# RmSchaffert/ACCV-Lab

Measured on AMD Instinct MI355X. Metric: heatmap frames/sec (1920x1080 fp32, ragged N_obj in [1,128], fused clear+draw), higher is better.
Workload: dtype f32

## Files before the change

### accv-lab_amd/accvlab/_amd_native/__init__.py

```python
from __future__ import annotations

import ctypes
import os

_HERE = os.path.dirname(os.path.abspath(__file__))
NO_HOST_FASTPATH = os.environ.get("ACCV_NO_HOST_FASTPATH", "") not in ("", "0")
LIB_PATH = os.environ.get("ACCV_HIP_LIB") or os.path.join(_HERE, "libaccv_hip.so")

OK = 0
HM_CLEAR = 1
HM_COUNTS_I64 = 2
HM_SMALL_RADII = 4
HM_WRITE_THROUGH = 8
HM_GROUP_BOXES_GIVEN = 16
HM_TILE_ROWS_16 = 32
HM_TILE_ROWS_8 = 64
HM_CALLER_SCALE_ORDER = 256
HM_PLAIN_STORES = 128
HM_POINT_COUNTS_I64 = 512
MP_IDX_I64 = 1
MP_COUNTS_I64 = 2
MP_LABELS_I64 = 4
FL_AVG_NUM_POS = 0
FL_AVG_VALUE = 1
FL_AVG_DEVICE = 2
LSA_MAXIMIZE = 1
LSA_THREADS_64 = 2
LSA_THREADS_1024 = 4
MC_ONE_MINUS_PROB = 0
MC_NEG_PROB = 1
MC_FOCAL = 2
MC_LABELS_I64 = 1
MC_CXCYWH = 2
CR_MAX_MAPS = 8
CR_MAX_CHANNELS = 64
CR_COUNTS_I64 = 1
CR_INDEX_FORM = 2
CR_WEIGHTS_PER_CHANNEL = 4
CR_L1 = 0
CR_SMOOTH_L1 = 2
MF_IDX_I64 = 1
MF_LABELS_I64 = 2
MB_IDX_I64 = 1
MB_CXCYWH = 2
MB_IOU_NONE = 0
MB_IOU = 1
MB_GIOU = 2
MB_MAX_D = 16
PM_IDX_I64 = 1
PM_REVERSIBLE = 2
PM_LABELS_I64 = 4
PM_CLOSED_I32 = 8
PM_CLOSED_I64 = 16
PM_MIN_P = 2
PM_MAX_P = 128
CT_MAX_TASKS = 8
CT_MAX_CLASSES = 64
CT_NO_TASK = 255
CT_LABELS_I64 = 1
CT_COUNTS_I64 = 2
BA_MAX_POINT_TRANSFORMS = 4
BA_MAX_FRAME_TRANSFORMS = 2
BA_COUNTS_I64 = 1
BA_LABELS_I64 = 2
BA_RANGE_ON_OUTPUT = 4
CD_MAX_TASKS = 8
CD_MAX_MAPS = 8
CD_MAX_CLASSES = 64
CD_MAX_K = 1024
RN_MAX_TASKS = 8
RN_MAX_N = 1024
RN_MIN_D = 7
RN_MAX_D = 16
VB_MAX_BOXES = 256
VB_COUNTS_I64 = 1
VB_HW_I64 = 2
CB_MAX_BOXES = 256
CB_MAX_MATRICES = 4
CB_COUNTS_I64 = 1
CB_HW_I64 = 2
CB_CATEGORIES_I64 = 4
BH_MAX_BOXES = 256
BH_MAX_CATEGORIES = 128
BH_TILE_W = 64
BH_TILE_H = 16
BH_COUNTS_I64 = 1
BH_HW_I64 = 2
BH_CATEGORIES_I64 = 4
IP_MAX_EXTENT = 16384
IP_TILE_W = 64
IP_TILE_H = 16
IP_LAYOUT_CHW = 0
IP_LAYOUT_HWC = 1

_vp = ctypes.c_void_p
_i = ctypes.c_int
_f = ctypes.c_float
_u = ctypes.c_uint
_sz = ctypes.c_size_t
_i64 = ctypes.c_int64
_ll = ctypes.c_longlong
_u64 = ctypes.c_uint64
# ... 381 lines not shown
```

### accv-lab_amd/accvlab/draw_heatmap/ops.py

```python
from __future__ import annotations

import ctypes
from typing import Optional

import torch

from .. import _amd_native as _nat

try:
    from . import _dh_host as _dh
except ImportError:
    _dh = None
_native_bound = False


def _native():
    global _native_bound
    if _dh is None or _nat.NO_HOST_FASTPATH:
        return None
    if not _native_bound:
        h = _nat.ctypes_lib()
        addr = lambda name: ctypes.cast(getattr(h, name), ctypes.c_void_p).value
        _dh.bind_native(addr("accv_draw_heatmap_batched_f32"), addr("accv_last_error"))
        _native_bound = True
    return _dh


_FORCED_FLAGS = 0


def _hint_flags(clear: bool, small_radii: bool, write_through: bool, tile_rows) -> int:
    if tile_rows not in (None, 8, 16):
        raise RuntimeError("tile_rows must be None, 8 or 16")
    return (_nat.HM_CLEAR if clear else 0) | (_nat.HM_SMALL_RADII if small_radii else 0) | \
        (0 if write_through is None else _nat.HM_WRITE_THROUGH if write_through else _nat.HM_PLAIN_STORES) | \
        (_nat.HM_TILE_ROWS_16 if tile_rows == 16 else _nat.HM_TILE_ROWS_8 if tile_rows == 8 else 0) | _FORCED_FLAGS


def _one_launch_maps(maps, batch: int, device):
    k = len(maps)
    if not 1 <= k <= 4:
        return None
    ptrs, hs, ws = [], [], []
    for hm in maps:
        if not (isinstance(hm, torch.Tensor) and hm.is_cuda and hm.dtype == torch.float32 and hm.is_contiguous() and
                hm.device == device):
            return None
        shape = hm.shape
        if len(shape) != 3 or shape[0] != batch:
            return None
        ptr = hm.data_ptr()
        if shape[2] % 4 or ptr % 16 or shape[1] * shape[2] * 4 >= (1 << 31):
            return None
        ptrs.append(ptr)
        hs.append(shape[1])
        ws.append(shape[2])
    return (ctypes.c_void_p * k)(*ptrs), (ctypes.c_int * k)(*hs), (ctypes.c_int * k)(*ws)


def _check_maps(maps, batch: int, device, owner: str) -> None:
    for hm in maps:
        _check_input(hm, "heatmap")
        _check_dtype(hm, torch.float32, "heatmap")
        if not (hm.dim() == 3 and hm.size(0) == batch):
            raise RuntimeError("every heatmap must be of shape [batch_size, height, width]")
        if not (hm.device == device):
            raise RuntimeError(f"every heatmap must be on the {owner}' device ({device})")


def _require(cond: bool, msg: str) -> None:
    if not cond:
        raise RuntimeError(msg)


def _check_input(t: torch.Tensor, name: str) -> None:
    if not (isinstance(t, torch.Tensor)):
        raise RuntimeError(f"{name} must be a torch.Tensor")
    if not (t.is_cuda):
        raise RuntimeError(f"{name} must be a CUDA tensor")
    if not (t.is_contiguous()):
        raise RuntimeError(f"{name} must be contiguous")


def _check_dtype(t: torch.Tensor, dtype: torch.dtype, name: str) -> None:
    if not (t.dtype == dtype):
        raise RuntimeError(f"{name}: expected scalar type {dtype} but found {t.dtype}")


def _same_device(ref: torch.Tensor, *others) -> None:
    for name, t in others:
        if not (t.device == ref.device):
            raise RuntimeError(f"{name} must be on the same device as the heatmap ({ref.device})")


_FLAT_DIRECT_MAX_OBJECTS = 2048
_FLAT_DIRECT_MAX_ROUNDS = 200_000
_constants: dict = {}


def _flat_direct(planes: int, height: int, width: int, n: int) -> bool:
    if not (0 < n <= _FLAT_DIRECT_MAX_OBJECTS and 0 < planes <= 65535 and height > 0 and width > 0):
        return False
    tiles = planes * ((width + 127) // 128) * ((height + 15) // 16)
    return tiles * ((n + 63) // 64) <= _FLAT_DIRECT_MAX_ROUNDS


def _device_constant(key, make) -> torch.Tensor:
    t = _constants.get(key)
    if t is None:
        t = make()
        if torch.cuda.is_current_stream_capturing():
            return t
        torch.cuda.current_stream(t.device).synchronize()
        if len(_constants) > 256:
            _constants.clear()
        _constants[key] = t
    return t


def draw_heatmap(
    heatmaps: torch.Tensor,
    centers: torch.Tensor,
    radii: torch.Tensor,
    heatmap_idxes: torch.Tensor,
    diameter_to_sigma_factor: float = 6.0,
    k_scale: float = 1.0,
    *,
    clear: bool = False,
    small_radii: bool = False,
    write_through: Optional[bool] = None,
    tile_rows: Optional[int] = None,
) -> None:
    _check_input(heatmaps, "heatmap")
    _check_input(centers, "centers")
    _check_input(radii, "radii")
    _check_input(heatmap_idxes, "heatmap_idxes")
    if not (centers.size(0) == radii.size(0)):
        raise RuntimeError("centers and radii must have the same size at dim0")
    if not (centers.size(0) == heatmap_idxes.size(0)):
        raise RuntimeError("centers and heatmap_idxes must have the same size at dim0")
    if not (heatmaps.dim() == 3):
        raise RuntimeError("heatmap must be of shape [num_heatmaps, height, width]")
    if not (centers.dim() == 2 and centers.size(1) == 2):
        raise RuntimeError("centers must be of shape [num_targets, 2]")
    if not (radii.dim() == 1 and heatmap_idxes.dim() == 1):
        raise RuntimeError("radii and heatmap_idxes must be of shape [num_targets]")
    _check_dtype(heatmaps, torch.float32, "heatmap")
    _check_dtype(centers, torch.int32, "centers")
    _check_dtype(radii, torch.int32, "radii")
    _check_dtype(heatmap_idxes, torch.int32, "heatmap_idxes")
    _same_device(heatmaps, ("centers", centers), ("radii", radii), ("heatmap_idxes", heatmap_idxes))

    lib = _nat.lib()
    planes, height, width = heatmaps.shape
    n = centers.size(0)
    if _flat_direct(planes, height, width, n):
        with _nat.device_guard(heatmaps.device):
            dev = heatmaps.device
            count = _device_constant(("count", n, dev), lambda: torch.full((1,), n, dtype=torch.int32, device=dev))
            status = lib.accv_draw_heatmap_batched_f32(
                heatmaps.data_ptr(), 1, planes, height, width, centers.data_ptr(), radii.data_ptr(), count.data_ptr(),
                heatmap_idxes.data_ptr(), n, float(diameter_to_sigma_factor), float(k_scale),
                _hint_flags(clear, small_radii, write_through, tile_rows), _nat.stream_ptr(heatmaps.device))
        _nat.check(status, "draw_heatmap")
        return
    with _nat.device_guard(heatmaps.device):
        ws_bytes = lib.accv_draw_heatmap_flat_workspace_bytes(planes, n)
        ws = torch.empty(ws_bytes, dtype=torch.uint8, device=heatmaps.device)
        status = lib.accv_draw_heatmap_flat_f32(
            heatmaps.data_ptr(), planes, height, width, centers.data_ptr(), radii.data_ptr(),
            heatmap_idxes.data_ptr(), n, float(diameter_to_sigma_factor), float(k_scale),
            _hint_flags(clear, small_radii, write_through, tile_rows), ws.data_ptr(), ws_bytes,
            _nat.stream_ptr(heatmaps.device))
    _nat.check(status, "draw_heatmap")


def draw_heatmap_batched(
    heatmap: torch.Tensor,
    centers,
    radii,
    diameter_to_sigma_factor: float = 6.0,
    k_scale: float = 1.0,
    labels=None,
    *,
    clear: bool = False,
    small_radii: bool = False,
    write_through: Optional[bool] = None,
    tile_rows: Optional[int] = None,
) -> None:
    centers_t = centers.tensor
    radii_t = radii.tensor
    assert centers_t.shape[0] == radii_t.shape[0], "centers and radii must have the same size batch size"
    assert centers_t.shape[1] == radii_t.shape[1], "centers and radii must have the same maximum number of objects"
    counts = centers.sample_sizes
    labels_t: Optional[torch.Tensor] = None
    if labels is not None:
        labels_t = labels.tensor
        assert centers_t.shape[0] == labels_t.shape[0], "centers and labels must have the same size batch size"
        assert centers_t.shape[1] == labels_t.shape[1], \
            "centers and labels must have the same maximum number of objects"

    native = _native()
    if native is not None and isinstance(heatmap, torch.Tensor) and isinstance(counts, torch.Tensor) and \
            native.draw_batched(heatmap, centers_t, radii_t, counts, labels_t, float(diameter_to_sigma_factor), float(k_scale),
                                _hint_flags(clear, small_radii, write_through, tile_rows)):
        return

    if counts.dtype not in (torch.int32, torch.int64):
        counts = counts.to(torch.int64)

    _check_input(heatmap, "heatmap")
    _check_input(centers_t, "centers")
    _check_input(radii_t, "radii")
    _check_input(counts, "nums_targets")
    batch = heatmap.size(0)
    n_max = radii_t.size(1) if radii_t.dim() >= 2 else -1
    _require(batch == radii_t.size(0) and batch == centers_t.size(0) and batch == counts.size(0),
             "batch_size (dim 0) need to be the same for all inputs")
    if not (centers_t.dim() == 3 and centers_t.size(2) == 2):
        raise RuntimeError("centers must be of shape [batch_size, num_targets, 2]")
    if not (radii_t.dim() == 2):
        raise RuntimeError("radii must be of shape [batch_size, num_targets]")
    if not (n_max == centers_t.size(1)):
        raise RuntimeError("maximum number of targets (dim 1) need to be the same centers and radii")
    if not (counts.dim() == 1):
        raise RuntimeError("nums_targets must be of shape [batch_size]")
    _check_dtype(heatmap, torch.float32, "heatmap")
    _check_dtype(centers_t, torch.int32, "centers")
    _check_dtype(radii_t, torch.int32, "radii")
    others = [("centers", centers_t), ("radii", radii_t), ("nums_targets", counts)]
    if labels_t is None:
        if not (heatmap.dim() == 3):
            raise RuntimeError("heatmap must be of shape [batch_size, height, width]")
        num_classes, (height, width) = 0, heatmap.shape[1:]
        labels_ptr = None
    else:
        _check_input(labels_t, "labels")
        if not (heatmap.dim() == 4):
            raise RuntimeError("heatmap must be of shape [batch_size, max_num_classes, height, width]")
        if not (labels_t.dim() == 2):
            raise RuntimeError("labels must be of shape [batch_size, radii.size(1)]")
        _require(labels_t.size(0) == batch and labels_t.size(1) == n_max,
                 "labels shape must be [batch_size, radii.size(1)]")
        _check_dtype(labels_t, torch.int32, "labels")
        num_classes, height, width = heatmap.shape[1:]
        if not (num_classes > 0 or heatmap.numel() == 0):
            raise RuntimeError("class-wise heatmap needs at least one class plane")
        labels_ptr = labels_t.data_ptr()
        others.append(("labels", labels_t))
    _same_device(heatmap, *others)
    if labels_t is not None and num_classes == 0:
        return

    flags = _hint_flags(clear, small_radii, write_through, tile_rows) | \
        (_nat.HM_COUNTS_I64 if counts.dtype == torch.int64 else 0)
    with _nat.device_guard(heatmap.device):
        status = _nat.lib().accv_draw_heatmap_batched_f32(
            heatmap.data_ptr(), batch, num_classes, height, width, centers_t.data_ptr(), radii_t.data_ptr(),
            counts.data_ptr(), labels_ptr, n_max, float(diameter_to_sigma_factor), float(k_scale), flags,
            _nat.stream_ptr(heatmap.device))
    _nat.check(status, "draw_heatmap_batched")


def get_centers_and_radii(centers, bboxes, out_size_factor: float):
    ragged = hasattr(centers, "tensor") and hasattr(centers, "create_with_sample_sizes_like_self")
    c_t = centers.tensor if ragged else centers
    b_t = bboxes.tensor if hasattr(bboxes, "tensor") else bboxes
    _require(c_t.shape[-1] == 2 and b_t.shape[-1] == 4 and c_t.shape[:-1] == b_t.shape[:-1],
             "centers must be [..., 2] and bboxes [..., 4] with equal leading dimensions")
    if c_t.is_cuda:
        if not (b_t.device == c_t.device):
            raise RuntimeError("centers and bboxes must be on the same device")
        c32 = c_t.to(torch.float32).contiguous()
        b32 = b_t.to(torch.float32).contiguous()
        out_c = torch.empty(c32.shape, dtype=torch.int32, device=c32.device)
        out_r = torch.empty(c32.shape[:-1], dtype=torch.int32, device=c32.device)
        with _nat.device_guard(c32.device):
            _nat.check(_nat.lib().accv_heatmap_targets_from_boxes_f32(
                c32.data_ptr(), b32.data_ptr(), out_r.numel(), float(out_size_factor), out_c.data_ptr(),
                out_r.data_ptr(), _nat.stream_ptr(c32.device)), "get_centers_and_radii")
    else:
        d = torch.cat([c_t - b_t[..., :2], b_t[..., 2:] - c_t], dim=-1)
        out_r = torch.ceil(torch.min(d, dim=-1)[0] / out_size_factor).to(torch.int32).clamp_(min=1)
        out_c = (c_t / out_size_factor).to(torch.int32)
    if ragged:
        nu = centers.non_uniform_dim
        return centers.create_with_sample_sizes_like_self(out_c, nu), centers.create_with_sample_sizes_like_self(out_r, nu)
    return out_c, out_r


def draw_heatmap_multiscale(heatmaps, centers, bboxes, out_size_factors, diameter_to_sigma_factor: float = 6.0,
                            k_scale: float = 1.0, *, clear: bool = False) -> None:
    heatmaps = list(heatmaps)
    strides = [float(f) for f in out_size_factors]
    if not (len(heatmaps) == len(strides) and len(heatmaps) >= 1):
        raise RuntimeError("heatmaps and out_size_factors must have the same, non-zero length")
    objects = _box_objects(centers, bboxes)
    batch, dev = objects[0].size(0), objects[0].device
    geometry = _one_launch_maps(heatmaps, batch, dev)
    if geometry is None:
        _check_maps(heatmaps, batch, dev, "centers")
        for hm, f in zip(heatmaps, strides):
            ci, ri = get_centers_and_radii(centers, bboxes, f)
            draw_heatmap_batched(hm, ci, ri, diameter_to_sigma_factor, k_scale, clear=clear)
        return
    _launch_box_maps(geometry, strides, objects, diameter_to_sigma_factor, k_scale, clear)


def _box_objects(centers, bboxes):
    c_t = centers.tensor
    b_t = bboxes.tensor if hasattr(bboxes, "tensor") else bboxes
    counts = centers.sample_sizes
    if counts.dtype not in (torch.int32, torch.int64):
        counts = counts.to(torch.int64)
    _check_input(c_t, "centers")
    _check_input(b_t, "bboxes")
    _check_input(counts, "nums_targets")
    if not (c_t.dim() == 3 and c_t.size(2) == 2):
        raise RuntimeError("centers must be of shape [batch_size, num_targets, 2]")
    if not (b_t.dim() == 3 and b_t.size(2) == 4 and b_t.shape[:2] == c_t.shape[:2]):
        raise RuntimeError("bboxes must be of shape [batch_size, num_targets, 4]")
    _check_dtype(c_t, torch.float32, "centers")
    _check_dtype(b_t, torch.float32, "bboxes")
    if not (counts.dim() == 1 and counts.size(0) == c_t.size(0)):
        raise RuntimeError("nums_targets must be of shape [batch_size]")
    _same_device(c_t, ("bboxes", b_t), ("nums_targets", counts))
    return c_t, b_t, counts


def _launch_box_maps(geometry, strides, objects, diameter_to_sigma_factor, k_scale, clear, job=None) -> None:
    ptrs, hs, ws = geometry
    c_t, b_t, counts = objects
    batch, n_max = c_t.shape[:2]
    n = len(strides)
    st = (ctypes.c_float * n)(*strides)
    flags = (_nat.HM_CLEAR if clear else 0) | (_nat.HM_COUNTS_I64 if counts.dtype == torch.int64 else 0) | _FORCED_FLAGS
    dev = c_t.device
# ... 13 lines not shown
```

### accv-lab_amd/csrc/draw_heatmap.hip

```cpp
#include <hip/hip_runtime.h>
#include <hip/hip_ext.h>

#include <algorithm>
#include <atomic>
#include <climits>
#include <cstdint>
#include <cstring>
#include <type_traits>

#include "accv_common.h"
#include "splat_common.h"
#include "splat_stamps.h"
#include "splat_tile.h"
#include "splat_small.h"
#include "splat_lanes.h"
#include "heatmap_prep.h"

namespace {

void note_dispatch(const char* kernel, int px, int r, bool clear, int sm, const dim3& grid, const dim3& block)
{
    snprintf(accv::dispatch_buffer(), 256, "%s<PX=%d,R=%d,CLEAR=%d,SM=%d> grid(%u,%u,%u) block(%u)", kernel, px, r, clear ? 1 : 0,
             sm, grid.x, grid.y, grid.z, block.x);
}

struct LaunchEvents {
    hipEvent_t start = nullptr, stop = nullptr;
};
LaunchEvents& launch_events()
{
    static thread_local LaunchEvents ev;
    return ev;
}
LaunchEvents take_launch_events()
{
    const LaunchEvents ev = launch_events();
    launch_events() = LaunchEvents{};
    return ev;
}
template <class K>
inline void launch_maybe_timed(K kernel, const dim3& grid, const dim3& block, hipStream_t stream, const LaunchEvents& ev,
                               const SplatParams& p)
{
    if (ev.start || ev.stop)
        hipExtLaunchKernelGGL(kernel, grid, block, 0, stream, ev.start, ev.stop, 0, p);
    else
        hipLaunchKernelGGL(kernel, grid, block, 0, stream, p);
}
template <class F>
void with_variant(bool clear, bool write_through, F&& f)
{
    using Plain = std::integral_constant<int, kStorePlain>;
    using WriteThrough = std::integral_constant<int, kStoreWriteThrough>;
    if (clear && write_through)
        f(std::true_type{}, WriteThrough{});
    else if (clear)
        f(std::true_type{}, Plain{});
    else if (write_through)
        f(std::false_type{}, WriteThrough{});
    else
        f(std::false_type{}, Plain{});
}

int launch_splat_small(SplatParams p, long long planes, bool clear, bool write_through, hipStream_t stream, const LaunchEvents& ev)
{
    p.tiles_x = (p.W + 127) / 128;
    p.tiles_y = (p.H + 15) / 16;
    p.n_tiles = planes * p.tiles_x * p.tiles_y;
    if (p.n_tiles == 0) return ACCV_OK;
    dim3 grid;
    p.grid3d = (planes <= 65535 && p.tiles_y <= 65535) ? 1 : 0;
    if (p.grid3d) {
        grid = dim3((unsigned)p.tiles_x, (unsigned)p.tiles_y, (unsigned)planes);
    } else {
        if (p.n_tiles > INT_MAX) return accv::fail(ACCV_EINVAL, "draw_heatmap: %lld tiles exceed the grid limit", p.n_tiles);
        grid = dim3((unsigned)p.n_tiles);
    }
    with_variant(clear, write_through, [&](auto CL, auto SM) {
        launch_maybe_timed(splat_small_kernel<CL, SM>, grid, dim3(64), stream, ev, p);
    });
    note_dispatch("splat_small_kernel", 4, 8, clear, write_through ? kStoreWriteThrough : kStorePlain, grid, dim3(64));
    return accv::check_launch("draw_heatmap small-splat kernel");
}

template <int PX, int R>
int launch_splat(SplatParams p, long long planes, bool clear, int sm, hipStream_t stream, const LaunchEvents& ev)
{
    p.tiles_x = (p.W + 32 * PX - 1) / (32 * PX);
    p.tiles_y = (p.H + 2 * R - 1) / (2 * R);
    p.n_tiles = planes * p.tiles_x * p.tiles_y;
    if (p.n_tiles == 0) return ACCV_OK;
    const int groups_x = (p.tiles_x + kWavesPerGroup - 1) / kWavesPerGroup;
    dim3 grid, block(kWavesPerGroup * 64);
    p.grid3d = (planes <= 65535 && p.tiles_y <= 65535) ? 1 : 0;
    if (p.grid3d) {
        grid = dim3((unsigned)groups_x, (unsigned)p.tiles_y, (unsigned)planes);
    } else {
        const long long groups = (p.n_tiles + kWavesPerGroup - 1) / kWavesPerGroup;
        if (groups > INT_MAX) return accv::fail(ACCV_EINVAL, "draw_heatmap: %lld tiles exceed the grid limit", p.n_tiles);
        grid = dim3((unsigned)groups);
    }
    attach_splat_stamps(p);
    if (PX == 1 || (sm == kStoreAdaptive && clear)) sm = kStorePlain;
    if (sm == kStoreAdaptive) {
        if constexpr (PX == 4) launch_maybe_timed(splat_kernel<PX, R, false, kStoreAdaptive>, grid, block, stream, ev, p);
    } else {
        with_variant(clear, sm == kStoreWriteThrough, [&](auto CL, auto SM) {
            if constexpr (PX == 4 || SM == kStorePlain) launch_maybe_timed(splat_kernel<PX, R, CL, SM>, grid, block, stream, ev, p);
        });
    }
    note_dispatch("splat_kernel", PX, R, clear, sm, grid, block);
    return accv::check_launch("draw_heatmap splat kernel");
}

long long compute_units()
{
    static std::atomic<int> cached[64];
    int dev = 0;
    if (hipGetDevice(&dev) != hipSuccess || dev < 0 || dev >= 64) return 0;
    int v = cached[dev].load(std::memory_order_relaxed);
    if (v == 0) {
        int n = 0;
        if (hipDeviceGetAttribute(&n, hipDeviceAttributeMultiprocessorCount, dev) != hipSuccess || n <= 0) return 0;
        cached[dev].store(n, std::memory_order_relaxed);
        v = n;
    }
    return v;
}

int dispatch_splat(SplatParams p, long long planes, bool clear, unsigned flags, hipStream_t stream, const LaunchEvents& ev)
{
    const bool small_hint = (flags & ACCV_HM_SMALL_RADII) != 0;
    const bool vec4 = (p.W % 4 == 0) && ((reinterpret_cast<uintptr_t>(p.hm) & 15u) == 0);
    const bool plane_fits_rsrc = (size_t)p.H * p.W * sizeof(float) < ((size_t)1 << 31);
    int nt;
    if (flags & ACCV_HM_WRITE_THROUGH)
        nt = kStoreWriteThrough;
    else if (flags & ACCV_HM_PLAIN_STORES)
        nt = kStorePlain;
    else
        nt = clear ? kStorePlain : kStoreAdaptive;
    if (nt != kStorePlain && !plane_fits_rsrc) nt = kStorePlain;
    p.dense_area = 0.75f * (float)p.H * (float)p.W;
    int rows = (flags & ACCV_HM_TILE_ROWS_16) ? 16 : 8;
    if (!(flags & (ACCV_HM_TILE_ROWS_8 | ACCV_HM_TILE_ROWS_16)) && clear && vec4 && !small_hint) {
        const long long cus = compute_units();
        const long long tx = (p.W + 127) / 128;
        const long long tiles8 = planes * tx * ((p.H + 15) / 16), tiles16 = planes * tx * ((p.H + 31) / 32);
        if (cus > 0 && tiles8 > 24 * cus && tiles16 <= 16 * cus) rows = 16;
    }
    if (!p.labels) p.labels = p.radii;
    if (!vec4) return launch_splat<1, 8>(p, planes, clear, kStorePlain, stream, ev);
    if (small_hint) return launch_splat_small(p, planes, clear, nt == kStoreWriteThrough, stream, ev);
    if (rows == 16) return launch_splat<4, 16>(p, planes, clear, nt, stream, ev);
    return launch_splat<4, 8>(p, planes, clear, nt, stream, ev);
}

int check_common(int h, int w, const char* who)
{
    if (h < 0 || w < 0) return accv::fail(ACCV_EINVAL, "%s: negative heatmap extent %dx%d", who, h, w);
    if (h > (1 << 29) || w > (1 << 29))
        return accv::fail(ACCV_EINVAL, "%s: heatmap extent %dx%d exceeds 2^29 per dimension", who, h, w);
    return ACCV_OK;
}

inline void coarse_scales_first(MultiParams& mp)
{
    std::stable_sort(mp.scale, mp.scale + mp.n_scales,
                     [](const SplatParams& a, const SplatParams& b) { return a.n_tiles < b.n_tiles; });
    long long tiles = 0;
    for (int i = 0; i < mp.n_scales; ++i) {
        mp.tile_begin[i] = tiles;
        tiles += mp.scale[i].n_tiles;
    }
    mp.tile_begin[mp.n_scales] = tiles;
}
inline void seal_tile_prefix(MultiParams& mp)
{
    for (int i = mp.n_scales + 1; i <= kMaxScales; ++i) mp.tile_begin[i] = mp.tile_begin[mp.n_scales];
}

inline int multiscale_store_mode(unsigned flags) { return (flags & ACCV_HM_WRITE_THROUGH) ? kStoreWriteThrough : kStorePlain; }

constexpr const char* kPerScaleNote = " (use the per-scale calls otherwise)";
long long setup_scales(MultiParams& mp, const SplatParams& proto, float* const* heatmaps, const int* heights, const int* widths,
                       const float* strides, int num_scales, int batch, int tile_h, unsigned flags, const char* who,
                       const char* map_note)
{
    long long tiles = 0;
    int used = 0;
    for (int i = 0; i < num_scales; ++i) {
        if (int rc = check_common(heights[i], widths[i], who)) return rc;
        if (!(strides[i] > 0.0f)) return accv::fail(ACCV_EINVAL, "%s: stride %d is not positive", who, i);
        if (heights[i] == 0 || widths[i] == 0) continue;
        if (!heatmaps[i]) return accv::fail(ACCV_EINVAL, "%s: heatmap %d is null", who, i);
        if (widths[i] % 4 != 0 || (reinterpret_cast<uintptr_t>(heatmaps[i]) & 15u) ||
            (size_t)heights[i] * widths[i] * sizeof(float) >= ((size_t)1 << 31))
            return accv::fail(ACCV_EINVAL, "%s: map %d needs a width that is a multiple of 4, a 16-byte aligned base and planes "
                                           "below 2 GiB%s", who, i, map_note);
        SplatParams& p = mp.scale[used];
        p = proto;
        p.hm = heatmaps[i];
        p.H = heights[i];
        p.W = widths[i];
        p.stride = strides[i];
        p.tiles_x = (p.W + 127) / 128;
        p.tiles_y = (p.H + tile_h - 1) / tile_h;
        p.n_tiles = (long long)batch * p.tiles_x * p.tiles_y;
        p.grid3d = 0;
        mp.tile_begin[used] = tiles;
        tiles += p.n_tiles;
        ++used;
    }
    mp.n_scales = used;
    mp.tile_begin[used] = tiles;
    if (!(flags & ACCV_HM_CALLER_SCALE_ORDER)) coarse_scales_first(mp);
    seal_tile_prefix(mp);
    return tiles;
}

int check_scale_arrays(const char* who, float* const* heatmaps, const int* heights, const int* widths, const float* strides,
                       int num_scales)
{
    if (num_scales < 1 || num_scales > kMaxScales)
        return accv::fail(ACCV_EINVAL, "%s: 1..%d scales supported, got %d", who, kMaxScales, num_scales);
    if (!heatmaps || !heights || !widths || !strides) return accv::fail(ACCV_EINVAL, "%s: null array", who);
    return ACCV_OK;
}
int check_scale_counts(const char* who, int batch, int per_sample, const char* what)
{
    if (batch < 0 || per_sample < 0) return accv::fail(ACCV_EINVAL, "%s: negative count", who);
    if (per_sample > (1 << 30)) return accv::fail(ACCV_EINVAL, "%s: more than 2^30 %s per sample", who, what);
    return ACCV_OK;
// ... 427 lines not shown
```

### accv-lab_amd/csrc/splat_common.h

```cpp
#pragma once
#include <hip/hip_runtime.h>

#include <cstdint>

#include "accv_common.h"

namespace {

constexpr int kWavesPerGroup = 1;
constexpr int kBoxTileR = 8;
constexpr int kCand = 64;
constexpr float kLog2e = 1.4426950408889634f;

constexpr int kSrcObjects = 0;
constexpr int kSrcFloatBoxes = 1;
constexpr int kSrcPoints = 2;
constexpr int kStorePlain = 0;
constexpr int kStoreWriteThrough = 4;
constexpr int kStoreAdaptive = 5;

struct SplatParams {
    float* hm;
    const int32_t* centers;
    const int32_t* radii;
    const int32_t* labels;
    const void* counts;
    const int32_t* plane_off;
    int H, W;
    int n_max;
    int n_classes;
    int tiles_x, tiles_y;
    long long n_tiles;
    float factor, k;
    int counts_i64;
    int grid3d;
    float dense_area;
    const float* centers_f;
    const float* boxes_f;
    float stride;
    int radius, n_groups;
#ifdef ACCV_SPLAT_STAMPS
    unsigned long long* stamps;
    long long stamp_records;
#endif
};

constexpr int kMaxScales = 4;
struct MultiParams {
    SplatParams scale[kMaxScales];
    long long tile_begin[kMaxScales + 1];
    int n_scales;
};

struct __attribute__((aligned(16))) Hit {
    int x, y;
    float c2;
    unsigned box;
};

template <int PX>
struct Vec;
typedef float vfloat4 __attribute__((ext_vector_type(4)));
template <>
struct Vec<4> {
    using type = vfloat4;
};
template <>
struct Vec<1> {
    using type = float;
};

__device__ __forceinline__ float raw_exp2(float x) { return __builtin_amdgcn_exp2f(x); }

__device__ __forceinline__ float max_skip_nan(float acc, float v)
{
    float r;
    asm("v_max_f32 %0, %1, %2" : "=v"(r) : "v"(acc), "v"(v));
    return r;
}

struct TileCtx {
    int tx0, ty0, tx1, ty1;
    long long plane;
    const int2* centers2;
    const int32_t* radii;
    const int32_t* labels;
    const float2* centers_f;
    const float4* boxes_f;
    float4 box0;
    float stride;
    int radius;
    int n, cls;
};

template <bool SCALAR_COUNT = false>
__device__ __forceinline__ void plane_objects(const SplatParams& p, TileCtx& t);

template <int TW, int TH, int WPG, bool SCALAR_COUNT = false>
__device__ __forceinline__ bool locate_tile(const SplatParams& p, int wave, TileCtx& t, long long linear_group)
{
    int tx, ty;
    if (p.grid3d) {
        tx = blockIdx.x * WPG + wave;
        ty = blockIdx.y;
        t.plane = blockIdx.z;
        if (tx >= p.tiles_x) return false;
    } else {
        const long long tile = linear_group * WPG + wave;
        if (tile >= p.n_tiles) return false;
        if (p.n_tiles <= 0x7fffffffll) {
            const unsigned t32 = (unsigned)tile, t2 = t32 / (unsigned)p.tiles_x;
            tx = (int)(t32 - t2 * (unsigned)p.tiles_x);
            const unsigned pl = t2 / (unsigned)p.tiles_y;
            ty = (int)(t2 - pl * (unsigned)p.tiles_y);
            t.plane = pl;
        } else {
            tx = (int)(tile % p.tiles_x);
            const long long t2 = tile / p.tiles_x;
            ty = (int)(t2 % p.tiles_y);
            t.plane = t2 / p.tiles_y;
        }
    }
    t.tx0 = tx * TW;
// ... 180 lines not shown
```

### accv-lab_amd/csrc/splat_stamps.h

```cpp
#pragma once

namespace {

template <bool ON>
struct PhaseStamps {
    __device__ __forceinline__ void start() {}
    __device__ __forceinline__ void cull() {}
    __device__ __forceinline__ void table() {}
    __device__ __forceinline__ void accumulate() {}
    __device__ __forceinline__ void record(const SplatParams&, long long, int, int, int) {}
};

#ifdef ACCV_SPLAT_STAMPS
constexpr bool kSplatStampsBuilt = true;
__device__ __forceinline__ unsigned long long phase_stamp()
{
    __builtin_amdgcn_sched_barrier(0);
    const unsigned long long v = __builtin_amdgcn_s_memrealtime();
    __builtin_amdgcn_sched_barrier(0);
    return v;
}
__device__ __forceinline__ unsigned xcc_id()
{
    unsigned v;
    asm volatile("s_getreg_b32 %0, hwreg(HW_REG_XCC_ID, 0, 4)" : "=s"(v));
    return v;
}

template <>
struct PhaseStamps<true> {
    unsigned long long st_start = 0, st_prev = 0, st_cull = 0, st_table = 0, st_acc = 0;
    int rounds = 0;

    __device__ __forceinline__ unsigned long long lap()
    {
        const unsigned long long now = phase_stamp(), d = now - st_prev;
        st_prev = now;
        return d;
    }
    __device__ __forceinline__ void start() { st_start = st_prev = phase_stamp(); }
    __device__ __forceinline__ void cull()
    {
        st_cull += lap();
        ++rounds;
    }
    __device__ __forceinline__ void table() { st_table += lap(); }
    __device__ __forceinline__ void accumulate() { st_acc += lap(); }
    __device__ __forceinline__ void record(const SplatParams& p, long long rec, int lane, int n, int total_hits)
    {
        const unsigned long long done = phase_stamp();
        if (lane == 0 && p.stamps && rec < p.stamp_records) {
            unsigned long long* o = p.stamps + 8 * rec;
            o[0] = st_start;
            o[1] = st_cull;
            o[2] = st_table;
            o[3] = st_acc;
            o[4] = st_prev;
            o[5] = (unsigned long long)n;
            o[6] = done;
            o[7] = (unsigned long long)(unsigned)total_hits | ((unsigned long long)rounds << 16) | ((unsigned long long)xcc_id() << 32);
        }
    }
};

unsigned long long* g_splat_stamps = nullptr;
long long g_splat_stamp_records = 0;
inline void attach_splat_stamps(SplatParams& p)
{
    p.stamps = g_splat_stamps;
    p.stamp_records = g_splat_stamp_records;
}
#else
constexpr bool kSplatStampsBuilt = false;
inline void attach_splat_stamps(SplatParams&) {}
#endif

}

#ifdef ACCV_SPLAT_STAMPS
extern "C" void accv_debug_splat_stamps(void* buffer, long long records)
{
    g_splat_stamps = static_cast<unsigned long long*>(buffer);
    g_splat_stamp_records = buffer ? records : 0;
}
#endif
```

### accv-lab_amd/csrc/splat_tile.h

```cpp
#pragma once

namespace {

template <int PX, int R, bool CLEAR, int SM, int WPG, int SRC>
__device__ __forceinline__ void splat_body(const SplatParams& p, long long linear_group)
{
    constexpr int kWavesPerGroup = WPG;
    constexpr int TW = 32 * PX;
    constexpr int TH = 2 * R;
    static_assert(R % 4 == 0, "row registers are fetched four at a time");

    __shared__ Hit s_hit[kWavesPerGroup][kCand];
    __shared__ __attribute__((aligned(16))) float s_ey[kWavesPerGroup][kCand][TH];

    constexpr bool kSharedColumns = CLEAR && SRC == kSrcObjects && PX == 4;
    PhaseStamps<kSplatStampsBuilt && CLEAR && SRC == kSrcObjects && PX == 4> stamps;
    stamps.start();
    const int lane = threadIdx.x & 63;
    const int wave = __builtin_amdgcn_readfirstlane(threadIdx.x >> 6);
    TileCtx t;
    if (!locate_tile<TW, TH, kWavesPerGroup>(p, wave, t, linear_group)) return;
    const int tx0 = t.tx0, ty0 = t.ty0, n = t.n;
    const long long plane = t.plane;

    const int sub = lane >> 5;
    const int col0 = tx0 + (lane & 31) * PX;

    float acc[R][PX];
    const float init = CLEAR ? 0.0f : __builtin_nanf("");
#pragma unroll
    for (int i = 0; i < R; ++i)
#pragma unroll
        for (int c = 0; c < PX; ++c) acc[i][c] = init;

    int total_hits = 0;
    float cover = 0.0f;

    for (int base = 0; base < n; base += kCand) {
        int x, y, r;
        const unsigned long long m = cull_round<SRC>(t, base, lane, x, y, r);
        if constexpr (SM == kStoreAdaptive) {
            const float dia = (float)(2 * min(max(r, 0), 1 << 20) + 1);
            cover += (base + lane < n) ? dia * dia : 0.0f;
        }
        const bool hit = (m >> lane) & 1ull;
        const int nh = __popcll(m);
        stamps.cull();
        if (nh == 0) continue;
        if constexpr (!CLEAR) {
            if (total_hits == 0 && col0 < p.W) {
                const float* plane_rd = p.hm + (size_t)plane * (size_t)p.H * (size_t)p.W;
#pragma unroll
                for (int i = 0; i < R; ++i) {
                    const int row = ty0 + sub * R + i;
                    if (row < p.H) {
                        if constexpr (PX == 4) {
                            const vfloat4 o = *reinterpret_cast<const vfloat4*>(plane_rd + (size_t)row * p.W + col0);
                            acc[i][0] = o.x;
                            acc[i][1] = o.y;
                            acc[i][2] = o.z;
                            acc[i][3] = o.w;
                        } else {
                            acc[i][0] = plane_rd[(size_t)row * p.W + col0];
                        }
                    }
                }
            }
        }
        if (hit) s_hit[wave][__popcll(m & ((1ull << lane) - 1ull))] = make_hit(p, t, x, y, r);
        __builtin_amdgcn_fence(__ATOMIC_RELEASE, "wavefront");
        __builtin_amdgcn_fence(__ATOMIC_ACQUIRE, "wavefront");

        for (int t = lane; t < nh * TH; t += 64) {
            const int h = t / TH, rr = t % TH;
            const Hit hy = s_hit[wave][h];
            const float d = (float)(ty0 + rr - hy.y);
            const float v = p.k * raw_exp2(-(d * d) * hy.c2);
            const unsigned ylo = (hy.box >> 16) & 255u, yhi = hy.box >> 24;
            s_ey[wave][h][rr] = ((unsigned)rr >= ylo && (unsigned)rr < yhi) ? v : __builtin_nanf("");
        }
        __builtin_amdgcn_fence(__ATOMIC_RELEASE, "wavefront");
        __builtin_amdgcn_fence(__ATOMIC_ACQUIRE, "wavefront");
        stamps.table();

        const unsigned colr0 = (unsigned)(lane & 31) * PX;
        auto column_factors = [&](const Hit& hx, float (&ex)[PX]) {
            const unsigned xlo = hx.box & 255u, xhi = (hx.box >> 8) & 255u;
#pragma unroll
            for (int c = 0; c < PX; ++c) {
                const float d = (float)(col0 + c - hx.x);
                const float e = raw_exp2(-(d * d) * hx.c2);
                ex[c] = (colr0 + c >= xlo && colr0 + c < xhi) ? e : __builtin_nanf("");
            }
        };
        [[maybe_unused]] auto column_factors_shared = [&](const Hit& hx, float (&ex)[PX]) {
            if constexpr (PX == 4) {
                const unsigned xlo = hx.box & 255u, xhi = (hx.box >> 8) & 255u;
                unsigned f[2];
#pragma unroll
                for (int j = 0; j < 2; ++j) {
                    const int c = 2 * sub + j;
                    const float d = (float)(col0 + c - hx.x);
                    const float e = raw_exp2(-(d * d) * hx.c2);
                    f[j] = __float_as_uint((colr0 + c >= xlo && colr0 + c < xhi) ? e : __builtin_nanf(""));
                }
#pragma unroll
                for (int j = 0; j < 2; ++j) {
                    const auto sw = __builtin_amdgcn_permlane32_swap(f[j], f[j], false, false);
                    ex[j] = __uint_as_float(sw[0]);
                    ex[2 + j] = __uint_as_float(sw[1]);
                }
            }
        };
        int h = 0;
        for (; CLEAR && h + 1 < nh; h += 2) {
            float exa[PX], exb[PX];
            if constexpr (kSharedColumns) {
                column_factors_shared(s_hit[wave][h], exa);
                column_factors_shared(s_hit[wave][h + 1], exb);
            } else {
                column_factors(s_hit[wave][h], exa);
                column_factors(s_hit[wave][h + 1], exb);
            }
#pragma unroll
            for (int q = 0; q < R / 4; ++q) {
                const float4 a4 = *reinterpret_cast<const float4*>(&s_ey[wave][h][sub * R + 4 * q]);
                const float4 b4 = *reinterpret_cast<const float4*>(&s_ey[wave][h + 1][sub * R + 4 * q]);
                const float eya[4] = {a4.x, a4.y, a4.z, a4.w}, eyb[4] = {b4.x, b4.y, b4.z, b4.w};
#pragma unroll
                for (int i = 0; i < 4; ++i)
#pragma unroll
                    for (int c = 0; c < PX; ++c)
                        acc[4 * q + i][c] = max3_skip_nan(acc[4 * q + i][c], exa[c] * eya[i], exb[c] * eyb[i]);
            }
        }
        for (; h < nh; ++h) {
            float ex[PX];
            if constexpr (kSharedColumns)
                column_factors_shared(s_hit[wave][h], ex);
            else
                column_factors(s_hit[wave][h], ex);
#pragma unroll
            for (int q = 0; q < R / 4; ++q) {
                const float4 e4 = *reinterpret_cast<const float4*>(&s_ey[wave][h][sub * R + 4 * q]);
                const float ey[4] = {e4.x, e4.y, e4.z, e4.w};
#pragma unroll
                for (int i = 0; i < 4; ++i)
#pragma unroll
                    for (int c = 0; c < PX; ++c) acc[4 * q + i][c] = max_skip_nan(acc[4 * q + i][c], ex[c] * ey[i]);
            }
        }
        total_hits += nh;
        stamps.accumulate();
        __builtin_amdgcn_fence(__ATOMIC_RELEASE, "wavefront");
        __builtin_amdgcn_fence(__ATOMIC_ACQUIRE, "wavefront");
    }

    if (!CLEAR && total_hits == 0) return;
    if (col0 >= p.W) return;

    using V = typename Vec<PX>::type;
    float* plane_ptr = p.hm + (size_t)plane * (size_t)p.H * (size_t)p.W;
    bool write_through = SM == kStoreWriteThrough;
    if constexpr (SM == kStoreAdaptive && PX == 4) {
#pragma unroll
        for (int d = 32; d >= 1; d >>= 1) cover += __shfl_xor(cover, d);
        write_through = cover >= p.dense_area;
    }
#pragma unroll
    for (int i = 0; i < R; ++i) {
        const int row = ty0 + sub * R + i;
        if (row >= p.H) break;
        V* dst = reinterpret_cast<V*>(plane_ptr + (size_t)row * p.W + col0);
        V out;
        if constexpr (PX == 4)
            out = V{acc[i][0], acc[i][1], acc[i][2], acc[i][3]};
        else
            out = acc[i][0];
        if constexpr (SM != kStorePlain && PX == 4) {
            if (write_through) {
                const auto rsrc = __builtin_amdgcn_make_buffer_rsrc(plane_ptr, 0, (int)((size_t)p.H * p.W * 4), 0x00020000);
                __builtin_amdgcn_raw_buffer_store_b128(out, rsrc, (int)(((size_t)row * p.W + col0) * 4), 0, 18);
            } else {
                *dst = out;
            }
        } else {
            *dst = out;
        }
    }
    stamps.record(p, (plane * p.tiles_y + ty0 / TH) * p.tiles_x + tx0 / TW, lane, n, total_hits);
}

template <int PX, int R, bool CLEAR, int SM, int WPG = kWavesPerGroup>
__global__ __launch_bounds__(WPG * 64) void splat_kernel(const SplatParams p)
{
    splat_body<PX, R, CLEAR, SM, WPG, kSrcObjects>(p, blockIdx.x);
}

template <bool CLEAR, int SM>
__global__ __launch_bounds__(64) void splat_multi_kernel(const MultiParams mp)
{
    long long first;
    const int s = scale_of_group(mp, blockIdx.x, first);
    splat_body<4, kBoxTileR, CLEAR, SM, 1, kSrcFloatBoxes>(mp.scale[s], (long long)blockIdx.x - first);
}

}
```

### include/accv_hip.h

```cpp
#ifndef ACCV_HIP_H
#define ACCV_HIP_H

#include <stddef.h>
#include <stdint.h>

#ifdef __cplusplus
extern "C" {
#endif

#define ACCV_OK 0
#define ACCV_EINVAL (-1)
#define ACCV_ELAUNCH (-2)
#define ACCV_EWORKSPACE (-3)
#define ACCV_ERUNTIME (-4)

#define ACCV_HM_CLEAR 1u
#define ACCV_HM_COUNTS_I64 2u
#define ACCV_HM_SMALL_RADII 4u
#define ACCV_HM_WRITE_THROUGH 8u
#define ACCV_HM_GROUP_BOXES_GIVEN 16u

#define ACCV_HM_PLAIN_STORES 128u
#define ACCV_HM_TILE_ROWS_16 32u
#define ACCV_HM_TILE_ROWS_8 64u
#define ACCV_HM_CALLER_SCALE_ORDER 256u

const char* accv_last_error(void);
int accv_version(void);
const char* accv_draw_heatmap_last_dispatch(void);


int accv_draw_heatmap_time_next_launch(void* start_event, void* stop_event);

size_t accv_draw_heatmap_flat_workspace_bytes(int num_planes, int num_objects);
int accv_draw_heatmap_flat_f32(float* heatmaps, int num_planes, int height, int width, const int32_t* centers,
                               const int32_t* radii, const int32_t* heatmap_idxes, int num_objects,
                               float diameter_to_sigma_factor, float k_scale, unsigned flags, void* workspace,
                               size_t workspace_bytes, void* stream);

int accv_draw_heatmap_batched_f32(float* heatmap, int batch, int num_classes, int height, int width,
                                  const int32_t* centers, const int32_t* radii, const void* counts,
                                  const int32_t* labels, int max_num_targets, float diameter_to_sigma_factor,
                                  float k_scale, unsigned flags, void* stream);

int accv_draw_heatmap_multiscale_f32(float* const* heatmaps, const int* heights, const int* widths, const float* strides,
                                     int num_scales, int batch, const float* centers_xy, const float* boxes_xyxy,
                                     const void* counts, int max_num_targets, float diameter_to_sigma_factor,
                                     float k_scale, unsigned flags, void* stream);

int accv_draw_heatmap_multiscale_sample_f32(float* const* heatmaps, const int* heights, const int* widths, const float* strides,
                                            int num_scales, int batch, const float* centers_xy, const float* boxes_xyxy,
                                            const void* counts, int max_num_targets, float diameter_to_sigma_factor,
                                            float k_scale, unsigned flags, const float* polylines_xy, int num_polylines,
                                            int points, const void* point_counts, int num_samples, float* samples,
                                            float* group_boxes, void* stream);

size_t accv_draw_points_workspace_bytes(int batch, int num_points);
int accv_draw_points_multiscale_f32(float* const* heatmaps, const int* heights, const int* widths, const float* strides,
                                    int num_scales, int batch, const float* points_xy, const void* counts, int num_points,
                                    int radius, float diameter_to_sigma_factor, float k_scale, unsigned flags,
                                    void* workspace, size_t workspace_bytes, void* stream);

#define ACCV_HM_POINT_COUNTS_I64 512u
int accv_draw_polylines_fused_applicable(const int* heights, const int* widths, int num_scales, int batch, int lanes,
                                         int points, int num_samples);
int accv_draw_polylines_multiscale_f32(float* const* heatmaps, const int* heights, const int* widths, const float* strides,
                                       int num_scales, int batch, const float* polylines_xy, int lanes, int points,
                                       const void* point_counts, const void* lane_counts, int num_samples, int radius,
                                       float diameter_to_sigma_factor, float k_scale, unsigned flags, void* stream);

int accv_heatmap_targets_from_boxes_f32(const float* centers_xy, const float* boxes_xyxy, long long num_objects,
                                        float stride, int32_t* out_centers, int32_t* out_radii, void* stream);

int accv_heatmap_targets_from_points_f32(const float* points_xy, long long num_points, float stride, int radius,
                                         int32_t* out_centers, int32_t* out_radii, void* stream);


int accv_ragged_gather(const void* src, void* dst, const void* indices, const void* counts, long long batch,
                       long long w_src, long long w_idx, long long idx_stride, long long row_bytes, int idx_i64,
                       int counts_i64, int* err_counter, void* stream);

int accv_ragged_gather_fill(const void* src, void* dst, const void* indices, const void* counts, long long batch,
                            long long w_src, long long w_idx, long long idx_stride, long long row_bytes,
                            uint64_t fill_bits, int elem_size, int idx_i64, int counts_i64, int* err_counter,
                            void* stream);

int accv_ragged_scatter(const void* src, void* dst, const void* indices, const void* counts, long long batch,
                        long long w_idx, long long idx_stride, long long w_dst, long long row_bytes, int idx_i64,
                        int counts_i64, int* err_counter, void* stream);

int accv_ragged_map_pairs(const void* src, void* dst, const void* src_indices, const void* dst_indices,
                          const void* counts, long long batch, long long w_src, long long w_idx, long long idx_stride,
                          long long w_dst, long long row_bytes, int idx_i64, int counts_i64, int* err_counter,
                          void* stream);

int accv_ragged_insert_const(void* dst, const void* indices, const void* counts, long long batch, long long w_idx,
                             long long idx_stride, long long w_dst, long long row_bytes, uint64_t elem_bits,
                             int elem_size, int idx_i64, int counts_i64, int* err_counter, void* stream);

int accv_ragged_pad_fill(void* data, const void* counts, long long batch, long long width, long long row_bytes,
                         uint64_t elem_bits, int elem_size, int counts_i64, void* stream);

int accv_ragged_accumulate(const void* src, void* dst, const void* src_indices_or_null, const void* dst_indices,
                           const void* counts, long long batch, long long w_src, long long w_idx, long long idx_stride,
                           long long w_dst, long long row_elems, int acc_dtype, int idx_i64, int counts_i64,
                           int* err_counter, void* stream);

int accv_ragged_mask_to_indices(const void* mask_u8, const void* valid_counts_or_null, int valid_i64, long long batch,
// ... 518 lines not shown
```

Baseline: 709,300.

## Prune dominated Gaussian hits per tile before accumulation in fused clear splat

Adds a per-tile pruning pass in the clear+vec4 splat path. For tiles with at least five candidate hits, it tests all pairs with a conservative dominance check (one Gaussian's max-blend can never exceed another's across the tile's box) and compacts the surviving hits in shared memory, so later per-pixel accumulation loops do less work. It also adds an amdgpu_waves_per_eu occupancy hint on the splat kernel and an opt-out flag. The risk is that the pairwise ballot overhead outweighs the savings on sparse tiles, and that the float bounds could be slightly inexact.

```diff
diff --git a/accv-lab_amd/accvlab/_amd_native/__init__.py b/accv-lab_amd/accvlab/_amd_native/__init__.py
--- a/accv-lab_amd/accvlab/_amd_native/__init__.py
+++ b/accv-lab_amd/accvlab/_amd_native/__init__.py
@@ -18,6 +18,7 @@
 HM_CALLER_SCALE_ORDER = 256
 HM_PLAIN_STORES = 128
 HM_POINT_COUNTS_I64 = 512
+HM_NO_PRUNE = 1024
 MP_IDX_I64 = 1
 MP_COUNTS_I64 = 2
 MP_LABELS_I64 = 4
diff --git a/accv-lab_amd/accvlab/draw_heatmap/ops.py b/accv-lab_amd/accvlab/draw_heatmap/ops.py
--- a/accv-lab_amd/accvlab/draw_heatmap/ops.py
+++ b/accv-lab_amd/accvlab/draw_heatmap/ops.py
@@ -29,12 +29,13 @@
 _FORCED_FLAGS = 0
 
 
-def _hint_flags(clear: bool, small_radii: bool, write_through: bool, tile_rows) -> int:
+def _hint_flags(clear: bool, small_radii: bool, write_through: bool, tile_rows, prune: bool = True) -> int:
     if tile_rows not in (None, 8, 16):
         raise RuntimeError("tile_rows must be None, 8 or 16")
     return (_nat.HM_CLEAR if clear else 0) | (_nat.HM_SMALL_RADII if small_radii else 0) | \
         (0 if write_through is None else _nat.HM_WRITE_THROUGH if write_through else _nat.HM_PLAIN_STORES) | \
-        (_nat.HM_TILE_ROWS_16 if tile_rows == 16 else _nat.HM_TILE_ROWS_8 if tile_rows == 8 else 0) | _FORCED_FLAGS
+        (_nat.HM_TILE_ROWS_16 if tile_rows == 16 else _nat.HM_TILE_ROWS_8 if tile_rows == 8 else 0) | \
+        (0 if prune else _nat.HM_NO_PRUNE) | _FORCED_FLAGS
 
 
 def _one_launch_maps(maps, batch: int, device):
@@ -130,6 +131,7 @@
     small_radii: bool = False,
     write_through: Optional[bool] = None,
     tile_rows: Optional[int] = None,
+    prune: bool = True,
 ) -> None:
     _check_input(heatmaps, "heatmap")
     _check_input(centers, "centers")
@@ -161,7 +163,7 @@
             status = lib.accv_draw_heatmap_batched_f32(
                 heatmaps.data_ptr(), 1, planes, height, width, centers.data_ptr(), radii.data_ptr(), count.data_ptr(),
                 heatmap_idxes.data_ptr(), n, float(diameter_to_sigma_factor), float(k_scale),
-                _hint_flags(clear, small_radii, write_through, tile_rows), _nat.stream_ptr(heatmaps.device))
+                _hint_flags(clear, small_radii, write_through, tile_rows, prune), _nat.stream_ptr(heatmaps.device))
         _nat.check(status, "draw_heatmap")
         return
     with _nat.device_guard(heatmaps.device):
@@ -170,7 +172,7 @@
         status = lib.accv_draw_heatmap_flat_f32(
             heatmaps.data_ptr(), planes, height, width, centers.data_ptr(), radii.data_ptr(),
             heatmap_idxes.data_ptr(), n, float(diameter_to_sigma_factor), float(k_scale),
-            _hint_flags(clear, small_radii, write_through, tile_rows), ws.data_ptr(), ws_bytes,
+            _hint_flags(clear, small_radii, write_through, tile_rows, prune), ws.data_ptr(), ws_bytes,
             _nat.stream_ptr(heatmaps.device))
     _nat.check(status, "draw_heatmap")
 
@@ -187,6 +189,7 @@
     small_radii: bool = False,
     write_through: Optional[bool] = None,
     tile_rows: Optional[int] = None,
+    prune: bool = True,
 ) -> None:
     centers_t = centers.tensor
     radii_t = radii.tensor
@@ -203,7 +206,7 @@
     native = _native()
     if native is not None and isinstance(heatmap, torch.Tensor) and isinstance(counts, torch.Tensor) and \
             native.draw_batched(heatmap, centers_t, radii_t, counts, labels_t, float(diameter_to_sigma_factor), float(k_scale),
-                                _hint_flags(clear, small_radii, write_through, tile_rows)):
+                                _hint_flags(clear, small_radii, write_through, tile_rows, prune)):
         return
 
     if counts.dtype not in (torch.int32, torch.int64):
@@ -252,7 +255,7 @@
     if labels_t is not None and num_classes == 0:
         return
 
-    flags = _hint_flags(clear, small_radii, write_through, tile_rows) | \
+    flags = _hint_flags(clear, small_radii, write_through, tile_rows, prune) | \
         (_nat.HM_COUNTS_I64 if counts.dtype == torch.int64 else 0)
     with _nat.device_guard(heatmap.device):
         status = _nat.lib().accv_draw_heatmap_batched_f32(
diff --git a/accv-lab_amd/csrc/draw_heatmap.hip b/accv-lab_amd/csrc/draw_heatmap.hip
--- a/accv-lab_amd/csrc/draw_heatmap.hip
+++ b/accv-lab_amd/csrc/draw_heatmap.hip
@@ -10,6 +10,7 @@
 
 #include "accv_common.h"
 #include "splat_common.h"
+#include "splat_prune_arith.h"
 #include "splat_stamps.h"
 #include "splat_tile.h"
 #include "splat_small.h"
@@ -149,6 +150,7 @@
         const long long tiles8 = planes * tx * ((p.H + 15) / 16), tiles16 = planes * tx * ((p.H + 31) / 32);
         if (cus > 0 && tiles8 > 24 * cus && tiles16 <= 16 * cus) rows = 16;
     }
+    p.prune = (!(flags & ACCV_HM_NO_PRUNE) && accv_prune::prune_allowed(p.k)) ? 1 : 0;
     if (!p.labels) p.labels = p.radii;
     if (!vec4) return launch_splat<1, 8>(p, planes, clear, kStorePlain, stream, ev);
     if (small_hint) return launch_splat_small(p, planes, clear, nt == kStoreWriteThrough, stream, ev);
diff --git a/accv-lab_amd/csrc/splat_common.h b/accv-lab_amd/csrc/splat_common.h
--- a/accv-lab_amd/csrc/splat_common.h
+++ b/accv-lab_amd/csrc/splat_common.h
@@ -39,6 +39,7 @@
     const float* boxes_f;
     float stride;
     int radius, n_groups;
+    int prune;
 #ifdef ACCV_SPLAT_STAMPS
     unsigned long long* stamps;
     long long stamp_records;
diff --git a/accv-lab_amd/csrc/splat_prune_arith.h b/accv-lab_amd/csrc/splat_prune_arith.h
--- /dev/null
+++ b/accv-lab_amd/csrc/splat_prune_arith.h
@@ -0,0 +1,59 @@
+#pragma once
+
+#if defined(__HIPCC__) || defined(__CUDACC__)
+#define ACCV_PRUNE_FN __host__ __device__ inline
+#define ACCV_PRUNE_ROLLED _Pragma("unroll 1")
+#else
+#define ACCV_PRUNE_FN inline
+#define ACCV_PRUNE_ROLLED
+#endif
+
+namespace accv_prune {
+
+constexpr float kDelta = 1.0e-3f;
+constexpr float kMaxExponent = 100.0f;
+constexpr float kPush = 1.0f / 262144.0f;
+constexpr float kMinK = 1.0f / 1048576.0f;
+
+ACCV_PRUNE_FN bool prune_allowed(float k) { return k >= kMinK && k <= 3.0e38f; }
+
+ACCV_PRUNE_FN float reciprocal(float v)
+{
+#if defined(__HIP_DEVICE_COMPILE__)
+    return __builtin_amdgcn_rcpf(v);
+#else
+    return 1.0f / v;
+#endif
+}
+
+ACCV_PRUNE_FN bool dominates(int ax, int ay, float ac2, unsigned abox, int bx, int by, float bc2, unsigned bbox, int tx0, int ty0)
+{
+    const unsigned range = ((unsigned)ax + 0x40000000u) | ((unsigned)ay + 0x40000000u) | ((unsigned)bx + 0x40000000u) |
+                           ((unsigned)by + 0x40000000u);
+    bool ok = abox != 0u && bbox != 0u && (range >> 31) == 0u && ac2 > 0.0f && bc2 > 0.0f && ac2 <= 3.0e38f && bc2 <= 3.0e38f;
+    const bool convex = bc2 > ac2;
+    const float cB_low = bc2 * (1.0f - kPush), cA_high = ac2 * (1.0f + kPush);
+    const float w = (ac2 * bc2) * reciprocal(bc2 - ac2) * (1.0f + kPush);
+    float bound = 0.0f, sq_a = 0.0f;
+    ACCV_PRUNE_ROLLED
+    for (int axis = 0; axis < 2; ++axis) {
+        const unsigned ab = axis ? abox >> 16 : abox, bb = axis ? bbox >> 16 : bbox;
+        const int tA = axis ? ay : ax, tB = axis ? by : bx, t0 = axis ? ty0 : tx0;
+        const int alo = (int)(ab & 255u), ahi = (int)((ab >> 8) & 255u), blo = (int)(bb & 255u), bhi = (int)((bb >> 8) & 255u);
+        ok = ok && alo <= blo && ahi >= bhi;
+        const int lo = t0 + blo, hi = t0 + bhi - 1;
+        const float dA0 = (float)(lo - tA), dA1 = (float)(hi - tA), dB0 = (float)(lo - tB), dB1 = (float)(hi - tB);
+        const float sA0 = dA0 * dA0, sA1 = dA1 * dA1;
+        sq_a += sA0 > sA1 ? sA0 : sA1;
+        const float f0 = cB_low * (dB0 * dB0) - cA_high * sA0, f1 = cB_low * (dB1 * dB1) - cA_high * sA1;
+        float m = f0 < f1 ? f0 : f1;
+        const float g0 = bc2 * dB0 - ac2 * dA0, g1 = bc2 * dB1 - ac2 * dA1;
+        const float dc = (float)(tA - tB);
+        const float v = -(w * (dc * dc));
+        m = (convex && g0 <= 0.0f && g1 >= 0.0f && v < m) ? v : m;
+        bound += m;
+    }
+    return ok && cA_high * sq_a <= kMaxExponent && bound >= kDelta;
+}
+
+}
diff --git a/accv-lab_amd/csrc/splat_stamps.h b/accv-lab_amd/csrc/splat_stamps.h
--- a/accv-lab_amd/csrc/splat_stamps.h
+++ b/accv-lab_amd/csrc/splat_stamps.h
@@ -6,6 +6,7 @@
 struct PhaseStamps {
     __device__ __forceinline__ void start() {}
     __device__ __forceinline__ void cull() {}
+    __device__ __forceinline__ void prune(int, int) {}
     __device__ __forceinline__ void table() {}
     __device__ __forceinline__ void accumulate() {}
     __device__ __forceinline__ void record(const SplatParams&, long long, int, int, int) {}
@@ -29,8 +30,8 @@
 
 template <>
 struct PhaseStamps<true> {
-    unsigned long long st_start = 0, st_prev = 0, st_cull = 0, st_table = 0, st_acc = 0;
-    int rounds = 0;
+    unsigned long long st_start = 0, st_prev = 0, st_cull = 0, st_table = 0, st_acc = 0, st_prune = 0;
+    int rounds = 0, hits_culled = 0, hits_pruned = 0;
 
     __device__ __forceinline__ unsigned long long lap()
     {
@@ -44,6 +45,12 @@
         st_cull += lap();
         ++rounds;
     }
+    __device__ __forceinline__ void prune(int before, int after)
+    {
+        st_prune += lap();
+        hits_culled += before;
+        hits_pruned += before - after;
+    }
     __device__ __forceinline__ void table() { st_table += lap(); }
     __device__ __forceinline__ void accumulate() { st_acc += lap(); }
     __device__ __forceinline__ void record(const SplatParams& p, long long rec, int lane, int n, int total_hits)
@@ -56,9 +63,10 @@
             o[2] = st_table;
             o[3] = st_acc;
             o[4] = st_prev;
-            o[5] = (unsigned long long)n;
+            o[5] = (unsigned long long)(unsigned)n | (st_prune << 32);
             o[6] = done;
-            o[7] = (unsigned long long)(unsigned)total_hits | ((unsigned long long)rounds << 16) | ((unsigned long long)xcc_id() << 32);
+            o[7] = (unsigned long long)(unsigned)total_hits | ((unsigned long long)rounds << 16) | ((unsigned long long)xcc_id() << 32) |
+                   ((unsigned long long)(hits_culled & 0xfff) << 40) | ((unsigned long long)(hits_pruned & 0xfff) << 52);
         }
     }
 };
diff --git a/accv-lab_amd/csrc/splat_tile.h b/accv-lab_amd/csrc/splat_tile.h
--- a/accv-lab_amd/csrc/splat_tile.h
+++ b/accv-lab_amd/csrc/splat_tile.h
@@ -14,6 +14,8 @@
     __shared__ __attribute__((aligned(16))) float s_ey[kWavesPerGroup][kCand][TH];
 
     constexpr bool kSharedColumns = CLEAR && SRC == kSrcObjects && PX == 4;
+    constexpr bool kPrune = CLEAR && SRC == kSrcObjects && PX == 4;
+    constexpr int kPruneMinHits = 5, kPruneAllPairs = R >= 16 ? 16 : 8;
     PhaseStamps<kSplatStampsBuilt && CLEAR && SRC == kSrcObjects && PX == 4> stamps;
     stamps.start();
     const int lane = threadIdx.x & 63;
@@ -44,7 +46,7 @@
             cover += (base + lane < n) ? dia * dia : 0.0f;
         }
         const bool hit = (m >> lane) & 1ull;
-        const int nh = __popcll(m);
+        int nh = __popcll(m);
         stamps.cull();
         if (nh == 0) continue;
         if constexpr (!CLEAR) {
@@ -70,6 +72,47 @@
         if (hit) s_hit[wave][__popcll(m & ((1ull << lane) - 1ull))] = make_hit(p, t, x, y, r);
         __builtin_amdgcn_fence(__ATOMIC_RELEASE, "wavefront");
         __builtin_amdgcn_fence(__ATOMIC_ACQUIRE, "wavefront");
+
+        if constexpr (kPrune) {
+            if (p.prune && nh >= kPruneMinHits) {
+                const int hits_before = nh;
+                const int blocks = (nh + 7) >> 3, a_blocks = nh <= kPruneAllPairs ? blocks : 1;
+                int pl = lane;
+                asm volatile("" : "+v"(pl));
+                const int la = pl >> 3, lb = pl & 7;
+                unsigned long long dead = 0ull;
+                for (int bb = 0; bb < blocks; ++bb) {
+                    const int b = bb * 8 + lb;
+                    const Hit hb = s_hit[wave][min(b, nh - 1)];
+                    unsigned dead8 = 0u;
+                    for (int ab = 0; ab < a_blocks; ++ab) {
+                        const int a = ab * 8 + la;
+                        const Hit ha = s_hit[wave][min(a, nh - 1)];
+                        const bool d = a < nh && b < nh &&
+                                       accv_prune::dominates(ha.x, ha.y, ha.c2, ha.box, hb.x, hb.y, hb.c2, hb.box, tx0, ty0);
+                        unsigned long long f = __ballot(d);
+                        f |= f >> 32;
+                        f |= f >> 16;
+                        f |= f >> 8;
+                        dead8 |= (unsigned)f & 255u;
+                    }
+                    dead |= (unsigned long long)dead8 << (8 * bb);
+                }
+                if (dead) {
+                    const unsigned long long alive = ~dead & (~0ull >> (64 - nh));
+                    typedef unsigned vuint4 __attribute__((ext_vector_type(4)));
+                    const vuint4 mine = *reinterpret_cast<const vuint4*>(&s_hit[wave][min(pl, nh - 1)]);
+                    __builtin_amdgcn_fence(__ATOMIC_RELEASE, "wavefront");
+                    __builtin_amdgcn_fence(__ATOMIC_ACQUIRE, "wavefront");
+                    if ((alive >> pl) & 1ull)
+                        *reinterpret_cast<vuint4*>(&s_hit[wave][__popcll(alive & ((1ull << pl) - 1ull))]) = mine;
+                    nh = __popcll(alive);
+                    __builtin_amdgcn_fence(__ATOMIC_RELEASE, "wavefront");
+                    __builtin_amdgcn_fence(__ATOMIC_ACQUIRE, "wavefront");
+                }
+                stamps.prune(hits_before, nh);
+            }
+        }
 
         for (int t = lane; t < nh * TH; t += 64) {
             const int h = t / TH, rr = t % TH;
@@ -191,8 +234,12 @@
     stamps.record(p, (plane * p.tiles_y + ty0 / TH) * p.tiles_x + tx0 / TW, lane, n, total_hits);
 }
 
+template <int PX, int R, bool CLEAR>
+constexpr int kSplatMinWaves = (CLEAR && PX == 4) ? (R == 8 ? 6 : R == 16 ? 4 : 1) : 1;
+
 template <int PX, int R, bool CLEAR, int SM, int WPG = kWavesPerGroup>
-__global__ __launch_bounds__(WPG * 64) void splat_kernel(const SplatParams p)
+__global__ __launch_bounds__(WPG * 64) __attribute__((amdgpu_waves_per_eu(kSplatMinWaves<PX, R, CLEAR>))) void splat_kernel(
+    const SplatParams p)
 {
     splat_body<PX, R, CLEAR, SM, WPG, kSrcObjects>(p, blockIdx.x);
 }
diff --git a/include/accv_hip.h b/include/accv_hip.h
--- a/include/accv_hip.h
+++ b/include/accv_hip.h
@@ -24,6 +24,7 @@
 #define ACCV_HM_TILE_ROWS_16 32u
 #define ACCV_HM_TILE_ROWS_8 64u
 #define ACCV_HM_CALLER_SCALE_ORDER 256u
+#define ACCV_HM_NO_PRUNE 1024u
 
 const char* accv_last_error(void);
 int accv_version(void);
```

Result: no change. 713,100 (median of 6 runs) (+0.5%).
